# k2kobayashi/crank

Hardware: AMD Instinct MI355X
Metric: train frames/sec (higher is better)
Workload: dtype bf16; 1 GPU; vqvae trainer step (all sub-updates), VCC2020-shaped synthetic 80-dim mlfb, 64 utterances x 500 frames per GPU, 14 speakers; trainer=vqvae, global_batch=64, batch_len=500, parallelism=dp1

## Files before the change

### crank_amd/_lib.py

```python
import ctypes
import os
from .config import cfg
from ctypes import c_char_p, c_double, c_float, c_int, c_longlong, c_ulonglong, c_void_p

_HERE = os.path.dirname(os.path.abspath(__file__))
LIB_PATH = cfg.lib_path or os.path.join(_HERE, "libcrank_hip.so")
_lib = None

ERRORS = {1: "invalid argument", 2: "HIP runtime error", 3: "unsupported shape/configuration"}


class NetDesc(ctypes.Structure):
    _fields_ = [
        ("kind", c_int), ("in_ch", c_int), ("out_ch", c_int), ("kernel_size", c_int), ("layers", c_int),
        ("stacks", c_int), ("res_ch", c_int), ("gate_ch", c_int), ("skip_ch", c_int), ("aux_ch", c_int),
        ("conv_ch", c_int), ("causal", c_int), ("use_bias", c_int), ("slope", c_float), ("dropout", c_float),
    ]


COLLATE_MAX_STREAMS = 8


class CollateStream(ctypes.Structure):
    _fields_ = [("src", c_void_p), ("ld", c_int), ("col0", c_int), ("ncols", c_int), ("dst", c_void_p)]
# ... 35 lines not shown
    "crk_net_conv_info": (I, [P, I, ctypes.POINTER(c_longlong)]),
    "crk_net_saved_bytes": (LL, [P, I, I]),
    "crk_net_reserve": (I, [P, I, I]),
    "crk_net_scratch_bytes": (LL, [P, I, I]),
    "crk_debug_alloc_count": (LL, []),
    "crk_debug_net_paths": (I, [P, I, I]),
    "crk_debug_net_partials": (LL, [P, I, I, P, LL, P]),
    "crk_seed_next": (I, [P, P, P]),
    "crk_nets_wnorm_bwd": (I, [I, P, P]),
    "crk_nets_prepare": (I, [I, P, P, ULL, P, P]),
    "crk_nets_prepare_models": (I, [I, P, P, P, I, P, P]),
    "crk_net_forward": (I, [P, P, ULL, P, I, P, I, P, I, P, I, I, I, ULL, P]),
    "crk_net_backward": (I, [P, P, ULL, P, P, I, P, I, P, I, P, I, F, P, I, P, I, I, I, ULL, P]),
    "crk_net_backward_scaled": (I, [P, P, ULL, P, P, I, P, I, P, I, P, I, F, P, I, P, I, I, I, ULL, P, P, P]),
    "crk_net_embed_grad_supported": (I, [P, I, I, I]),
    "crk_net_backward_embed": (I, [P, P, ULL, P, P, I, P, I, P, I, P, I, F, P, I, I, I, ULL, P, LL, I, I, I, P, P]),
    "crk_vq_forward": (I, [P, I, P, I, I, I, P, P, I, P, I, P]),
    "crk_vq_forward_fused": (I, [P, I, P, I, P, I, P, I, I, I, P, P, I, P, I, P, P, P, P, P]),
    "crk_vq_image_bytes": (LL, [I, I]),
    "crk_vq_image_build_multi": (I, [I, P, P, I, P, P]),
    "crk_vq_ema_scratch_bytes": (LL, [I, I, I]),
    "crk_vq_ema_stats": (I, [P, I, P, I, I, I, P, P, P, P]),
    "crk_vq_ema_apply": (I, [P, P, P, P, P, I, I, D, D, P]),
    "crk_vq_ema_partial": (I, [P, I, P, I, I, I, P, P]),
    "crk_vq_ema_reduce_multi": (I, [I, P, P, P, P, P, P, P]),
    "crk_vq_ema_apply_multi": (I, [I, P, P, P, P, P, P, P, D, D, P]),
    "crk_vq_ema_partial_multi": (I, [I, P, P, P, P, P, P, P, P]),
    "crk_vq_ema_reduce_size_multi": (I, [I, P, P, P, P, P, P, P, D, D, P]),
    "crk_vq_ema_blend_multi": (I, [I, P, P, P, P, P, P, D, P]),
    "crk_vq_ema_blend_image_multi": (I, [I, P, P, P, P, P, P, D, P, P]),
# ... 152 lines not shown
```

### crank_amd/config.py

```python
import contextlib
import os
import types

_get = os.environ.get


def _flag(name, default):
    v = _get(name)
    return default if v is None else v not in ("0", "")


def _read():
    return types.SimpleNamespace(
        precision=_get("CRANK_AMD_PRECISION", "bf16"),
        lib_path=_get("CRANK_AMD_LIB") or None,
        default_yaml=_get("CRANK_DEFAULT_YAML") or None,
        overlap_c=int(_get("CRANK_AMD_OVERLAP_C", "3") or 0),
        separate_ce=_flag("CRANK_AMD_SEPARATE_CE", False),
        separate_commit=_flag("CRANK_AMD_SEPARATE_COMMIT", False),
        recon_dense=_flag("CRANK_AMD_RECON_DENSE", False),
        stft_two_pass=_flag("CRANK_AMD_STFT_TWO_PASS", False),
        cond_sums=_flag("CRANK_AMD_COND_SUMS", True),
        force_dist=_flag("CRANK_AMD_FORCE_DIST", False),
        dist_backend=_get("CRANK_AMD_DIST_BACKEND") or None,
        dp_graph_collectives=_flag("CRANK_AMD_DP_GRAPH_COLLECTIVES", True),
        capture_mode=_get("CRANK_AMD_CAPTURE_MODE", "thread_local"),
        test_refuse_capture_rank=_get("CRANK_AMD_TEST_REFUSE_CAPTURE_RANK"),
    )


cfg = _read()


def reload():
    cfg.__dict__.update(_read().__dict__)


# ... 17 lines not shown
```

### crank_amd/csrc/conv_kernels.h

```cpp
#pragma once
#include <vector>

#include "runtime.h"

#define CRK_TM 128

enum { MODE_PLAIN = 0, MODE_RESFWD = 1, MODE_BWDA = 2 };

struct ConvP {
  const float* xa; int lda; int cinA; float scaleA;
  const float* xb; int ldb; int cinB; float scaleB;
  int act_in; float slope;
  float drop_p; unsigned long long drop_seed;
  const unsigned long long* drop_seed_ptr;
  int cin, cin_pad;
  const float* xc; int ldc; int cinC; int cinC_pad;
  const uint16_t* w_hi; const uint16_t* w_lo;
  const uint16_t* wc_hi; const uint16_t* wc_lo;
  const uint16_t* w2_hi; const uint16_t* w2_lo;
  const float* bias; const float* bias2a; const float* bias2b;
  int cout, cout_pad, ktaps, dil, off0;
  int B, T, tiles_per_utt;
  float* y; int ldy; int accumulate; int act_out; float out_scale;
  const float* dmask; int ldm; int dmask_act;
// ... 61 lines not shown
  float drop_p; unsigned long long drop_seed; const unsigned long long* drop_seed_ptr;
  int o_xlo, o_zhi, o_zlo, o_chi, o_clo, o_whi, o_wlo, o_bias, o_tab, w_bytes, lds_bytes;
  int nw;
  int dbg;
  int ft, fh;
  int ft1;
  int o_zs, o_cs;
  int o_xf;
  const float* x_in; int ldx_in, in_ch, kp_first;
  long long f_first, b_first;
  long long f_h1, b_h1, f_h2, b_h2;
  float* y; int ldy, out_ch; float head_scale;
  uint16_t* fin_hi; uint16_t* head_hi;
  long long ts_stride;
  int cs_stride;
};
struct PsLayer {
  long long w_off;
  long long b_off;
  int rows, rows_pad;
  int kp;
  int k, dil, off0;
  int epi;
  int mask_w;
  long long mask_plane;
  long long save_plane;
  long long f_off;
};
struct PsP {
  const float* x; int ldx, cin; float in_scale; int in_act;
// ... 133 lines not shown
```

### crank_amd/csrc/net.hip

```cpp
#include <math.h>
#include <stdlib.h>
#include <string.h>

#include <deque>
#include <vector>

#include "conv_kernels.h"

#include "../../include/crank_hip.h"

enum { ROLE_FIRST = 0, ROLE_CONV = 1, ROLE_AUX = 2, ROLE_OUT = 3, ROLE_SKIP = 4, ROLE_LAST1 = 5, ROLE_LAST2 = 6, ROLE_PLAIN = 7 };

struct ConvMeta {
  int role, layer, dilation;
};

static bool g_may_alloc = false;
static long long g_net_allocs = 0;
static hipError_t net_malloc_(void** p, size_t bytes) {
  if (!g_may_alloc) return hipErrorInvalidValue;
  g_net_allocs++;
  return hipMalloc(p, bytes);
}
#define NET_MALLOC(pp, bytes) net_malloc_(reinterpret_cast<void**>(pp), (bytes))
// ... 632 lines not shown
    if (t.saved != saved) continue;
    if (t.B == B && t.T == T && t.mode == want && (want != 2 || t.x3f == expects_x3f)) {
      if (t.fused == fused) return CRK_OK;
      fprintf(stderr, "[crank_hip] crk_net_backward: the %s kernels would read a workspace the %s forward wrote (flags 0x%x, B %d, T %d)\n",
              fused ? "fused" : "per-layer", t.fused ? "fused" : "per-layer", flags, B, T);
      return CRK_ERR_ARG;
    }
    fprintf(stderr, "[crank_hip] crk_net_backward: flags 0x%x (plane layout %d%s, B %d, T %d) do not match the forward that wrote this "
                    "workspace (layout %d%s, B %d, T %d): CRK_FLAG_PRECISE pairs with CRK_FLAG_PRECISE, CRK_FLAG_PRECISE | CRK_FLAG_BWD_PLAIN "
                    "with CRK_FLAG_FWD_PRECISE, plain with plain\n", flags, want, expects_x3f ? " x3f" : "", B, T, t.mode, t.x3f ? " x3f" : "", t.B, t.T);
    return CRK_ERR_ARG;
  }
  return CRK_OK;
}

struct FwdIo {
  const float* params; const float* x; int ldx; const float* c; int ldc; float* y; int ldy; float* saved; int B, T; hipStream_t s;
};
enum { FWD_CHAIN, FWD_CHAIN_LAYERS, FWD_FOLDED, FWD_FUSED, FWD_LAYERS };
static int fwd_form(const Net* n, const Route& rt, const Call& k, bool x3f, int* form) {
  if (n->d.kind == 2) { *form = rt.fused ? FWD_CHAIN : FWD_CHAIN_LAYERS; return CRK_OK; }
  const bool io16 = k.in16 && k.out16;
  if ((x3f || rt.gen_split) && !io16) {
    fprintf(stderr, "[crank_hip] crk_net_forward: x / y must be 16-byte aligned with row strides that are multiples of 4 floats\n");
    return CRK_ERR_ARG;
  }
  if (x3f || (rt.fold_fwd && io16)) *form = FWD_FOLDED;
  else if (rt.gen_split) return CRK_ERR_UNSUPPORTED;
  else *form = rt.fused ? FWD_FUSED : FWD_LAYERS;
  return CRK_OK;
}

// ... 50 lines not shown
  sp.xb_lo = b16 + gf.xb_lo; sp.zb_lo = b16 + gf.zb_lo; sp.tb_lo = b16 + gf.tb_lo; sp.sg_lo = b16 + gf.sg_lo;
  if (n->d.aux_ch > 0) sp.cb_lo = b16 + gf.cb_lo;
  return sp;
}
static int fwd_folded(const Net* n, const Route& rt, const Call& k, const FwdIo& a, bool x3f) {
  const crk_net_desc& d = n->d;
  const ConvEntry& ef = n->ents[n->idx_first];
  const ConvEntry& e1 = n->ents[n->idx_last1];
  const ConvEntry& e2 = n->ents[n->idx_last2];
  StackP sp = stack_fwd_params(n, k, a, false);
  sp.x_in = a.x; sp.ldx_in = a.ldx; sp.in_ch = d.in_ch; sp.kp_first = ef.fw_kp;
  sp.f_first = ef.fr_off; sp.b_first = ef.off_b;
  sp.f_h1 = e1.fr_off; sp.b_h1 = e1.off_b; sp.f_h2 = e2.fr_off; sp.b_h2 = e2.off_b;
  sp.y = a.y; sp.ldy = a.ldy; sp.out_ch = d.out_ch; sp.head_scale = (float)sqrt(1.0 / n->L);
  if (x3f || rt.gen_split) sp.ts_stride = ts_plane_stride((long long)a.B * a.T);
  if (x3f) { RUN(stack2x_fwd_plan(sp)); return launch_stack2x_fwd(sp, a.s); }
  RUN(stack2_fwd_plan(sp));
  return launch_stack2_fwd(sp, a.s);
}
static int fwd_fused(const Net* n, const Shape* r, const Call& k, const FwdIo& a) {
  const crk_net_desc& d = n->d;
  const Route& rt = r->route[k.precise];
  const long long N = (long long)a.B * a.T;
  const GatedF32 lay = gated_f32(n, N);
  const GatedB16 gf = gated_b16(n, N);
  uint16_t* b16 = reinterpret_cast<uint16_t*>(a.saved + saved_f32_floats(n, N));
  PsP f = ps_base(n, a.B, a.T, a.params);
  f.x = a.x; f.ldx = a.ldx; f.cin = d.in_ch; f.y = a.saved + lay.x; f.ldy = 64; f.L = 1;
  if (k.keep) { f.save_hi = b16 + gf.f_hi; f.save_lo = b16 + gf.f_lo; }
  RUN(pstack_go(r, 0, f, k.precise, a.s));
// ... 37 lines not shown
    }
    p.w2_hi = n->whi + eo.fw_off; p.w2_lo = n->wlo + eo.fw_off;
    p.bias2a = eo.off_b >= 0 ? a.params + eo.off_b : nullptr;
    p.bias2b = es.off_b >= 0 ? a.params + es.off_b : nullptr;
    p.skip = SKIP; p.skip_init = (l == 0);
    p.sv_ta = a.saved + lay.ta + l * P; p.sv_sb = a.saved + lay.sb + l * P; p.sv_z = a.saved + lay.z + l * P;
    RUN(conv_go(p, MODE_RESFWD, k.precise, a.s));
  }
  ConvP h1 = conv_fw(n, a.B, a.T, n->ents[n->idx_last1], a.params, SKIP, 64, H1, 64);
  h1.scaleA = (float)sqrt(1.0 / L); h1.act_in = head_act;
  RUN(conv_go(h1, MODE_PLAIN, k.precise, a.s));
  ConvP h2 = conv_fw(n, a.B, a.T, n->ents[n->idx_last2], a.params, H1, 64, a.y, a.ldy);
  h2.act_in = head_act;
  return conv_go(h2, MODE_PLAIN, k.precise, a.s);
}
extern "C" int crk_net_forward(void* h, const float* params, unsigned long long version, const float* x, int ldx,
                               const float* c, int ldc, float* y, int ldy, float* saved, int B, int T, int flags,
                               unsigned long long seed, void* stream) {
  Net* n = (Net*)h;
  if (!n || !params || !x || !y || B <= 0 || T <= 0) return CRK_ERR_ARG;
  const FwdIo a = {.params = params, .x = x, .ldx = ldx, .c = c, .ldc = ldc, .y = y, .ldy = ldy, .saved = saved, .B = B, .T = T,
                   .s = (hipStream_t)stream};
  const Call k = call_facts(flags, seed, true, x, ldx, y, ldy, nullptr, nullptr);
  const Shape* r = find_shape(n, B, T);
  if (!r) return not_reserved("crk_net_forward");
  const Route rt = call_route(r, k);
  const bool x3f = k.mode == 2 && r->route[0].x3f;
  RUN(ensure_prepared(n, params, version, a.s));
  if (n->d.kind != 2 && (!saved || (n->d.aux_ch > 0 && !c))) return CRK_ERR_ARG;
  int form;
  RUN(fwd_form(n, rt, k, x3f, &form));
  tag_forward(n, saved, B, T, k, x3f, form != FWD_LAYERS && form != FWD_CHAIN_LAYERS);
  switch (form) {
    case FWD_CHAIN: return fwd_chain(n, r, k, a);
    case FWD_CHAIN_LAYERS: return fwd_chain_layers(n, k, a);
    case FWD_FOLDED: return fwd_folded(n, rt, k, a, x3f);
    case FWD_FUSED: return fwd_fused(n, r, k, a);
  }
  return fwd_layers(n, k, a);
}

static int stack_cpg(const Net* n, int B, int T) {
  const int ncpu = (T + 63) / 64;
  const int groups = crk_sw().wg_groups;
  const int gsz = (B + groups - 1) / groups;
  int cpg = gsz * ncpu;
  if (crk_sw().wg_fill && n->d.kind != 2 && n->L > 0 && 256 / n->L > groups) {
    const int fill = 256 / n->L;
    const int c = (B * ncpu + fill - 1) / fill;
    if (c >= 1 && c < cpg) cpg = c;
  }
  return cpg < 1 ? 1 : cpg;
}
static int stack_groups(const Net* n, int B, int T) {
// ... 597 lines not shown
```

### crank_amd/csrc/stack2_kernels.hip

```cpp
#include "conv_kernels.h"

#include "stack_common.h"

#define S2_NCU 256
#define S2_PAIR_FACTOR 1.0


template <int KT, int AKC, int FT, int R, int FH, bool DROP, bool FOLD>
__device__ __forceinline__ void s2_wave(const StackP& p, unsigned char* smem, const int rb) {
  constexpr int XS = SK_XS, NT = 256 * FH;
  const int tid = threadIdx.x, lane = tid & 63, l31 = lane & 31, half = lane >> 5;
  const int wave = __builtin_amdgcn_readfirstlane(tid >> 6);
  const int mt = wave & 3, fh = FH > 1 ? wave >> 2 : 0;
  const bool res_wave = mt < 2;
  const int b = blockIdx.x / p.tiles_per_utt, tile = blockIdx.x - b * p.tiles_per_utt;
  const int t0 = tile * p.tmo;
  const long nbase = (long)b * p.T;
  const long P = (long)p.B * p.T * 64;
  SK_PROF_BEGIN()

  unsigned char* xs = smem;
  unsigned char* zs = smem + p.o_zs;
  unsigned char* cs = smem + p.o_cs;
  StackLayer* lay_s = reinterpret_cast<StackLayer*>(smem + p.o_tab);
  float* bias_s = reinterpret_cast<float*>(smem + p.o_bias);

  int row[FT], voff_st[FT], voff_b[FT];
  unsigned rmask[FT];
  bool rin[FT];
  const bool save_b = p.xb_hi != nullptr;
  const int ch_st = 32 * (mt & 1) + 4 * half;
#pragma unroll
  for (int ft = 0; ft < FT; ft++) {
    row[ft] = rb + ft * 32 + l31;
// ... 28 lines not shown
      xq[u] = __builtin_amdgcn_raw_buffer_load_b128(rxi, on ? (int)(((nbase + t) * p.ldx_in + c4) * 4) : SK_OOB, 0, 0);
      xrow += xdr; xcol += xdc;
      if (xcol >= ppr) { xcol -= ppr; xrow++; }
    }
    if (res_wave) {
      const int KF = p.kp_first >> 4;
#pragma unroll
      for (int kc = 0; kc < 8; kc++) awf[kc] = S2_WLOAD(p.f_first + (mt * KF + (kc < KF ? kc : 0)) * 512);
    }
#pragma unroll
    for (int q = 0; q < 4; q++)
      bfq[q] = (res_wave && p.b_first >= 0) ? *reinterpret_cast<const sk_f32x4*>(p.params + p.b_first + 32 * mt + 8 * q + 4 * half) : sk_f32x4{0.f, 0.f, 0.f, 0.f};
  }
  constexpr int CNQ = R * 16, CPER = AKC > 0 ? (CNQ + NT - 1) / NT : 1;
  float av[CPER][4];
  if (AKC > 0) {
#pragma unroll
    for (int it = 0; it < CPER; it++) {
      const int idx = tid + it * NT, r = idx >> 4, c4 = (idx & 15) << 2;
      const int tt = t0 - p.hl + r;
      const bool on = idx < CNQ && tt >= 0 && tt < p.T;
      const long n = nbase + tt;
#pragma unroll
      for (int j = 0; j < 4; j++) av[it][j] = (on && c4 + j < p.aux_ch) ? p.c[n * p.ldc + c4 + j] : 0.f;
    }
  }
  SK_T(12)
  constexpr int NBI = 16 * 256 / NT;
  float bv[NBI];
#pragma unroll
  for (int k = 0; k < NBI; k++) {
// ... 427 lines not shown
  } else if (!res_wave) {
    const __amdgpu_buffer_rsrc_t r_sk = sk_rsrc(p.skip, P);
#pragma unroll
    for (int ft = 0; ft < FT; ft++)
#pragma unroll
      for (int q = 0; q < 4; q++) {
        sk_u32x4 v;
#pragma unroll
        for (int j = 0; j < 4; j++) v[j] = sk_f2u(st[ft][4 * q + j]);
        __builtin_amdgcn_raw_buffer_store_b128(v, r_sk, voff_st[ft] + q * 32, 0, 0);
      }
  }
  SK_PROF_END(7)
}

template <int KT, int AKC, int FT, int FH, bool DROP, bool FOLD, int FT1 = FT>
__global__ __launch_bounds__(256 * FH, 2) void stack2_fwd_kernel(const StackP p) {
  extern __shared__ __attribute__((aligned(16))) unsigned char smem[];
  constexpr int R = FH > 1 ? 32 * (FT + FT1) : 32 * FT;
  const int fh = FH > 1 ? __builtin_amdgcn_readfirstlane((int)threadIdx.x >> 8) : 0;
  if constexpr (FT1 == FT) {
    s2_wave<KT, AKC, FT, R, FH, DROP, FOLD>(p, smem, fh * 32 * FT);
  } else {
    if (fh == 0) s2_wave<KT, AKC, FT, R, FH, DROP, FOLD>(p, smem, 0);
    else s2_wave<KT, AKC, FT1, R, FH, DROP, FOLD>(p, smem, 32 * FT);
  }
}

int stack2_fwd_plan(StackP& p) {
  if ((p.ktaps != 3 && p.ktaps != 5) || p.max_off > SK_GUARD || p.aux_ch > 64 || p.L > 16) return CRK_ERR_UNSUPPORTED;
  if (p.ktaps == 3 && p.aux_ch > 0) return CRK_ERR_UNSUPPORTED;
  static int cfg_env = -1;
  if (cfg_env < 0) cfg_env = crk_sw().s2_cfg;
  static const int shapes[3][3] = {{2, 2, 2}, {3, 2, 2}, {3, 2, 3}};
  int best = -1; double best_cost = 0;
  for (int i = 0; i < 3; i++) {
    const int ft = shapes[i][0], fh = shapes[i][1], ft1 = shapes[i][2];
    const int code = ft1 == ft ? ft * 10 + fh : (ft * 10 + fh) * 10 + ft1;
    if (cfg_env && cfg_env != code) continue;
    if (ft1 != ft && (p.ktaps != 3 || p.drop_p > 0.f)) continue;
// ... 13 lines not shown
  p.tmo = ceil_div(p.T, p.tiles_per_utt);
  int off = (SK_GUARD * 2 + R) * SK_XS;
  p.o_zs = off; off += R * SK_XS;
  p.o_cs = off; if (p.aux_ch > 0) off += R * SK_XS;
  p.o_bias = off; off += p.L * 256 * 4;
  p.o_tab = off; off += p.L * (int)sizeof(StackLayer);
  off = (off + 15) & ~15;
  if (p.x_in) {
    if (p.kp_first < 16 || p.kp_first > 128 || (p.kp_first & 15)) return CRK_ERR_UNSUPPORTED;
    p.o_xf = off; off += R * (p.kp_first * 2 + 16);
  }
  p.lds_bytes = (off + 15) & ~15;
  return p.lds_bytes <= (p.fh == 1 ? 80 : 160) * 1024 ? CRK_OK : CRK_ERR_UNSUPPORTED;
}

template <int KT, int AKC, bool DROP, bool FOLD>
static int s2_launch_shape(const StackP& p, dim3 grid, hipStream_t s) {
#define S2_GO(FTV, FHV)                                                                                              \
  {                                                                                                                  \
    CRK_RAISE_LDS_ONCE(160 * 1024, stack2_fwd_kernel<KT, AKC, FTV, FHV, DROP, FOLD>)                                 \
    hipLaunchKernelGGL((stack2_fwd_kernel<KT, AKC, FTV, FHV, DROP, FOLD>), grid, dim3(256 * FHV), p.lds_bytes, s, p);       \
  }
  if (p.ft == 2) S2_GO(2, 2) else if (p.ft1 == 0) S2_GO(3, 2)
  else if constexpr (KT == 3 && !DROP) {
    CRK_RAISE_LDS_ONCE(160 * 1024, stack2_fwd_kernel<KT, AKC, 3, 2, DROP, FOLD, 2>)
    hipLaunchKernelGGL((stack2_fwd_kernel<KT, AKC, 3, 2, DROP, FOLD, 2>), grid, dim3(512), p.lds_bytes, s, p);
  } else return CRK_ERR_UNSUPPORTED;
#undef S2_GO
  return CRK_OK;
}

int launch_stack2_fwd(const StackP& p, hipStream_t s) {
  dim3 grid(p.B * p.tiles_per_utt);
  const double nfr = (double)p.B * p.T;
  conv_prof_bytes(1, nfr * (256.0 + 4.0 * p.aux_ch + 256.0 + (p.xb_hi ? 512.0 * p.L + 2.0 * (p.aux_ch > 0 ? p.aux_pad : 0) : 0.0)));
  conv_prof_begin(1, 2.0 * nfr * (p.L * (128.0 * (64.0 * p.ktaps + p.aux_ch) + 128.0 * 64.0) +
                                   (p.x_in ? 64.0 * p.in_ch + 64.0 * 64.0 + 64.0 * p.out_ch : 0.0)), s);
  const int akc = p.aux_ch > 0 ? (p.aux_ch + 15) / 16 : 0;
  int rc = CRK_OK;
  const bool fold = p.x_in != nullptr;
#define S2_DISPATCH(KTV, AKCV) (fold ? s2_launch_shape<KTV, AKCV, false, true>(p, grid, s) : s2_launch_shape<KTV, AKCV, false, false>(p, grid, s))
  if (p.ktaps == 3) rc = S2_DISPATCH(3, 0);
  else if (p.drop_p > 0.f) {
    if (akc || fold) return CRK_ERR_UNSUPPORTED;
    rc = s2_launch_shape<5, 0, true, false>(p, grid, s);
  } else if (akc == 0) rc = S2_DISPATCH(5, 0);
  else if (akc == 1) rc = S2_DISPATCH(5, 1);
  else if (akc <= 3) rc = S2_DISPATCH(5, 3);
  else rc = S2_DISPATCH(5, 4);
#undef S2_DISPATCH
  conv_prof_end(1, s);
  if (rc != CRK_OK) return rc;
  CRK_CHECK_LAUNCH();
  return CRK_OK;
}
```

### crank_amd/net/module/vqvae2.py

```python
import torch

from ... import ops, parallel
from .flat import FlatModel
from .mlfb import LogMelFilterBankLayer
from .pwg import KIND_GENERATOR, MAX_CHANNELS, HipStack


class Quantizer:

    def __init__(self, owner, prefix, emb_dim, emb_size, decay=0.99, eps=1e-5, ema_flag=False, bdt_flag=False):
        self.owner, self.prefix = owner, prefix
        self.emb_dim, self.emb_size = emb_dim, emb_size
        self.decay, self.eps, self.ema_flag, self.bdt_flag = decay, eps, ema_flag, bdt_flag
        self.cb_offset = None
        self.training = True
        self.bucket, self.slot = None, 0
        self._img, self._img_epoch = None, -1

    def entries(self, base):
        self.cb_offset = base
        return [(self.prefix + "embedding.weight", base, (self.emb_size, self.emb_dim))]

    @property
    def n_params(self):
# ... 275 lines not shown
            q.training = mode
        return self

    @property
    def spkr_table(self):
        o = self.emb_offset
        return self.flat.data[o: o + self.spkr_size * self.emb_size].view(self.spkr_size, self.emb_size)

    def spkr_embedding(self, h):
        return ops.concat_embed(None, None, self.spkr_table, h, self, self.emb_offset, self.flat)

    def _get_dec_h(self, dec_h, spkrvec):
        a, b = dec_h if isinstance(dec_h, (tuple, list)) else (dec_h, None)
        if spkrvec is not None:
            if torch.is_grad_enabled() and ops.embed_owned_ok(self.decoders[0].net, a, b, spkrvec):
                return ops.concat_embed_owned(a, b, self.spkr_table, spkrvec, self, self.emb_offset)
            return ops.concat_embed(a, b, self.spkr_table, spkrvec, self, self.emb_offset, self.flat)
        return dec_h if b is None else torch.cat([a, b], dim=-1)

    def _pre(self, x):
        return self.preprocess_layer(x) if self.conf["use_raw"] else x

    def encode(self, x, enc_h=None):
        out = []
        cur = x
        dims = self.conf["emb_dim"][: self.conf["n_vq_stacks"]]
        ebuf = torch.empty(x.shape[0], x.shape[1], sum(dims), device=x.device, dtype=torch.float32)
        col = 0
        for n in range(self.conf["n_vq_stacks"]):
            cur = self.encoders[n](cur, c=enc_h if n == 0 else None, out=(ebuf, col))
            col += dims[n]
# ... 103 lines not shown
```

### crank_amd/ops.py

```python
import ctypes

import torch

from . import _lib
from .config import cfg
from ._lib import check, ptr, stream_ptr

_PRECISION = cfg.precision


def set_precision(name):
    global _PRECISION
    if name not in ("bf16", "bf16x3", "bf16x3f"):
        raise ValueError(f"unknown precision {name!r} (bf16 | bf16x3 | bf16x3f)")
    _PRECISION = name


def get_precision():
    return _PRECISION


CRK_FLAG_PRECISE = 1
CRK_FLAG_NO_PARAM_GRAD = 2
CRK_FLAG_NO_SAVE = 4
# ... 95 lines not shown
        key = (B, T, _PRECISION)
        v = self._saved_bytes.get(key)
        if v is None:
            check(_lib.lib().crk_net_reserve(self.handle, B, T), "crk_net_reserve")
            v = self._saved_bytes[key] = _lib.lib().crk_net_saved_bytes(self.handle, B, T)
        return v

    def embed_grad_supported(self, B, T):
        key = ("embed", B, T, _PRECISION)
        v = self._saved_bytes.get(key)
        if v is None:
            self.saved_bytes(B, T)
            v = self._saved_bytes[key] = bool(_lib.lib().crk_net_embed_grad_supported(self.handle, B, T, _flags(backward=True)))
        return v

    def __del__(self):
        try:
            if getattr(self, "handle", None):
                _lib.lib().crk_net_destroy(self.handle)
                self.handle = None
        except Exception:
            pass


class _NetFn(torch.autograd.Function):

    @staticmethod
    def forward(ctx, x, c, flat, net, owner, offset, dx_scale, no_save=False, ybuf=None, ycol=0, emb=None):
        L = _lib.lib()
        B, T = x.shape[0], x.shape[1]
        if emb is not None and not (c is not None and emb.run == T and net.embed_grad_supported(B, T)):
            raise RuntimeError("conditioning built by concat_embed_owned fed to a net that cannot own its table gradient")
        xk, ldx = _rows(x)
        ck, ldc = (None, 0) if c is None else _rows(c)
        if ybuf is None:
            y = torch.empty(B, T, net.out_ch, device=x.device, dtype=torch.float32)
        else:
            y = ybuf[..., ycol: ycol + net.out_ch]
        ldy = y.stride(1)
        nbytes = net.saved_bytes(B, T)
        saved = torch.empty(max(nbytes // 4, 1), device=x.device, dtype=torch.float32)
        seed_t = net.next_seed() if net.dropout > 0 else None
        params = flat.data_ptr() + 4 * offset
        check(
            L.crk_net_forward(net.handle, params, owner.version, ptr(xk), ldx, ptr(ck), ldc, ptr(y), ldy,
                              ptr(saved), B, T, _flags(no_save=no_save) | (CRK_FLAG_SEED_ON_DEVICE if seed_t is not None else 0), ptr(seed_t),
                              stream_ptr()),
            "crk_net_forward",
        )
        ctx.net, ctx.owner, ctx.offset, ctx.dx_scale, ctx.seed = net, owner, offset, dx_scale, seed_t
        ctx.precision = _PRECISION
        ctx.ld = (ldx, ldc)
        ctx.version = owner.version
        ctx.save_for_backward(xk, ck if ck is not None else torch.empty(0, device=x.device), flat)
        ctx.saved_ws = saved
        ctx.has_c = c is not None
        ctx.emb = emb
        return y

    @staticmethod
    def backward(ctx, dy):
        L = _lib.lib()
        net, owner = ctx.net, ctx.owner
        xk, ck, flat = ctx.saved_tensors
# ... 751 lines not shown
                  "crk_weighted_sum_bwd")
        return (None, None) + tuple(grads[i] for i in range(len(ws)))


def weighted_sum(terms, weights, constant=0.0):
    return _WeightedSumFn.apply(tuple(weights), float(constant), *terms)


def _label_runs(idx):
    B, T = idx.shape
    if T > 1 and idx.stride(1) == 0 and (B == 1 or idx.stride(0) == T):
        return idx, T
    return idx.contiguous(), 1


def _concat_embed_fwd(a, b, table, idx):
    L = _lib.lib()
    B, T = idx.shape
    ak, lda = (None, 0) if a is None else _rows(a)
    bk, ldb = (None, 0) if b is None else _rows(b)
    ca = 0 if a is None else a.shape[-1]
    cb = 0 if b is None else b.shape[-1]
    E = table.shape[1]
    out = torch.empty(B, T, ca + cb + E, device=idx.device, dtype=torch.float32)
    ik, run = _label_runs(idx)
    check(L.crk_concat_embed_run(ptr(ak), lda, ca, ptr(bk), ldb, cb, ptr(table), E, ptr(ik), run, B * T, ptr(out),
                                 ca + cb + E, stream_ptr()), "crk_concat_embed_run")
    return out, ik, run, (ca, cb, E)


class _ConcatEmbedFn(torch.autograd.Function):

    @staticmethod
    def forward(ctx, a, b, table, idx, owner, tab_offset, flat):
        out, ik, run, (ca, cb, E) = _concat_embed_fwd(a, b, table, idx)
        B, T = idx.shape
        ctx.geom = (ca, cb, E, table.shape[0], run, B * T)
        ctx.owner, ctx.tab_offset = owner, tab_offset
        ctx.save_for_backward(ik)
        return out

    @staticmethod
    def backward(ctx, dout):
# ... 5 lines not shown
            ctx.owner.grads_clean = False
            g = ctx.owner.grad_flat[ctx.tab_offset: ctx.tab_offset + rows * E]
            scratch = torch.empty(L.crk_embed_bwd_scratch_floats(N, E, rows), device=dk.device, dtype=torch.float32)
            check(L.crk_embed_bwd_run(ptr(dk), ld, ca + cb, E, ptr(ik), run, N, rows, ptr(g), ptr(scratch), stream_ptr()),
                  "crk_embed_bwd_run")
        da = dk[..., :ca] if (ca and ctx.needs_input_grad[0]) else None
        db = dk[..., ca:ca + cb] if (cb and ctx.needs_input_grad[1]) else None
        return da, db, None, None, None, None, None


def concat_embed(a, b, table, idx, owner=None, tab_offset=0, flat=None):
    return _ConcatEmbedFn.apply(a, b, table, idx, owner, tab_offset, flat)


class EmbedCond:
    __slots__ = ("idx", "run", "c0", "E", "rows", "owner", "tab_offset")


def embed_owned_ok(net, a, b, idx):
    if not cfg.cond_sums or idx.dim() != 2:
        return False
    if (a is not None and a.requires_grad) or (b is not None and b.requires_grad):
        return False
    B, T = idx.shape
    return _label_runs(idx)[1] == T and net.embed_grad_supported(B, T)


def concat_embed_owned(a, b, table, idx, owner, tab_offset):
    with torch.no_grad():
        out, ik, run, (ca, cb, E) = _concat_embed_fwd(a, b, table, idx)
    e = EmbedCond()
    e.idx, e.run, e.c0, e.E, e.rows, e.owner, e.tab_offset = ik, run, ca + cb, E, table.shape[0], owner, tab_offset
    out._crk_embed = e
    return out


def adam_step(flat, grad, exp_avg, exp_avg_sq, lr_dev, step_dev, beta1=0.9, beta2=0.999, eps=1e-8, clear_grads=False,
              defer_bump=False):
    check(_lib.lib().crk_adam_step(ptr(flat), ptr(grad), ptr(exp_avg), ptr(exp_avg_sq), flat.numel(), ptr(lr_dev),
                                   ptr(step_dev), beta1, beta2, eps, (1 if clear_grads else 0) | (2 if defer_bump else 0),
                                   stream_ptr()), "crk_adam_step")


def adam_step_multi(blocks, beta1=0.9, beta2=0.999, eps=1e-8, clear_grads=False, defer_bump=False):
    rec = (_lib.AdamBlock * len(blocks))()
    for r, (flat, grad, m, v, lr_dev, step_dev) in zip(rec, blocks):
# ... 38 lines not shown
```

### include/crank_hip.h

```cpp
#ifndef CRANK_HIP_H
#define CRANK_HIP_H
#ifdef __cplusplus
extern "C" {
#endif

#define CRK_OK 0
#define CRK_ERR_ARG 1
#define CRK_ERR_HIP 2
#define CRK_ERR_UNSUPPORTED 3

#define CRK_FLAG_PRECISE 1
#define CRK_FLAG_NO_PARAM_GRAD 2
#define CRK_FLAG_NO_SAVE 4
#define CRK_FLAG_DEFER_WNORM 8

#define CRK_FLAG_SEED_ON_DEVICE 16
#define CRK_FLAG_FWD_PRECISE 32
#define CRK_FLAG_BWD_PLAIN 64

typedef struct crk_net_desc {
  int kind;
  int in_ch, out_ch, kernel_size, layers, stacks;
  int res_ch, gate_ch, skip_ch, aux_ch;
  int conv_ch;
// ... 2 lines not shown
  float slope;
  float dropout;
} crk_net_desc;

void* crk_net_create(const crk_net_desc* desc);
void crk_net_destroy(void* net);
long long crk_net_param_count(void* net);
int crk_net_conv_count(void* net);
int crk_net_conv_info(void* net, int i, long long* out9);
long long crk_net_saved_bytes(void* net, int B, int T);
int crk_net_reserve(void* net, int B, int T);
long long crk_net_scratch_bytes(void* net, int B, int T);
int crk_net_forward(void* net, const float* params, unsigned long long version, const float* x, int ldx,
                    const float* c, int ldc, float* y, int ldy, float* saved, int B, int T, int flags,
                    unsigned long long seed, void* stream);
int crk_net_backward(void* net, const float* params, unsigned long long version, float* grads, const float* x,
                     int ldx, const float* c, int ldc, const float* dy, int lddy, float* dx, int lddx, float dx_scale,
                     float* dc, int lddc, const float* saved, int B, int T, int flags, unsigned long long seed,
                     void* stream);
int crk_net_backward_scaled(void* net, const float* params, unsigned long long version, float* grads, const float* x,
                            int ldx, const float* c, int ldc, const float* dy, int lddy, float* dx, int lddx, float dx_scale,
                            float* dc, int lddc, const float* saved, int B, int T, int flags, unsigned long long seed,
                            const float* dy_num, const float* dy_den, void* stream);
int crk_net_embed_grad_supported(void* net, int B, int T, int flags);
int crk_net_backward_embed(void* net, const float* params, unsigned long long version, float* grads, const float* x, int ldx,
                           const float* c, int ldc, const float* dy, int lddy, float* dx, int lddx, float dx_scale,
                           const float* saved, int B, int T, int flags, unsigned long long seed, const long long* idx,
                           long long run, int c0, int E, int n_rows, float* dtable, void* stream);

int crk_seed_next(unsigned long long* state, unsigned long long* out, void* stream);
// ... 304 lines not shown
```

Before: 22.51 million frames/s.

## Fuse speaker-embedding concat gather into stacked decoder forward kernel

Instead of materializing the concatenated conditioning tensor (encoder outputs plus speaker embedding) with a separate concat kernel, the decoder's folded stack2 forward kernel now reads the two encoder parts and the embedding table row directly when it loads aux inputs. A placeholder NaN-expanded tensor stands in for the unbuilt conditioning, and the code falls back to the explicit concat when the gather path is unsupported. This removes one kernel launch and a B*T*aux_ch write/read, at the cost of a new template instantiation, extra per-element branching in the aux load, and risk if any consumer touches the placeholder tensor.

Result: no change. 22.48 million frames/s (median of 2 runs) (-0.1%).

```diff
diff --git a/crank_amd/_lib.py b/crank_amd/_lib.py
--- a/crank_amd/_lib.py
+++ b/crank_amd/_lib.py
@@ -73,6 +73,8 @@
     "crk_net_backward": (I, [P, P, ULL, P, P, I, P, I, P, I, P, I, F, P, I, P, I, I, I, ULL, P]),
     "crk_net_backward_scaled": (I, [P, P, ULL, P, P, I, P, I, P, I, P, I, F, P, I, P, I, I, I, ULL, P, P, P]),
     "crk_net_embed_grad_supported": (I, [P, I, I, I]),
+    "crk_net_forward_embed": (I, [P, P, ULL, P, I, P, I, I, P, I, I, P, I, P, LL, I, P, I, P, I, I, I, ULL, P]),
+    "crk_net_embed_gather_supported": (I, [P, I, I, I]),
     "crk_net_backward_embed": (I, [P, P, ULL, P, P, I, P, I, P, I, P, I, F, P, I, I, I, ULL, P, LL, I, I, I, P, P]),
     "crk_vq_forward": (I, [P, I, P, I, I, I, P, P, I, P, I, P]),
     "crk_vq_forward_fused": (I, [P, I, P, I, P, I, P, I, I, I, P, P, I, P, I, P, P, P, P, P]),
diff --git a/crank_amd/config.py b/crank_amd/config.py
--- a/crank_amd/config.py
+++ b/crank_amd/config.py
@@ -21,6 +21,7 @@
         recon_dense=_flag("CRANK_AMD_RECON_DENSE", False),
         stft_two_pass=_flag("CRANK_AMD_STFT_TWO_PASS", False),
         cond_sums=_flag("CRANK_AMD_COND_SUMS", True),
+        cond_gather=_flag("CRANK_AMD_COND_GATHER", True),
         force_dist=_flag("CRANK_AMD_FORCE_DIST", False),
         dist_backend=_get("CRANK_AMD_DIST_BACKEND") or None,
         dp_graph_collectives=_flag("CRANK_AMD_DP_GRAPH_COLLECTIVES", True),
diff --git a/crank_amd/csrc/conv_kernels.h b/crank_amd/csrc/conv_kernels.h
--- a/crank_amd/csrc/conv_kernels.h
+++ b/crank_amd/csrc/conv_kernels.h
@@ -99,6 +99,8 @@
   uint16_t* fin_hi; uint16_t* head_hi;
   long long ts_stride;
   int cs_stride;
+  const float* c2; int ldc2, ca, cb;
+  const float* emb_table; const long long* emb_idx; long long emb_run; int emb_c0, emb_E, emb_rows;
 };
 struct PsLayer {
   long long w_off;
diff --git a/crank_amd/csrc/net.hip b/crank_amd/csrc/net.hip
--- a/crank_amd/csrc/net.hip
+++ b/crank_amd/csrc/net.hip
@@ -670,8 +670,10 @@
   return CRK_OK;
 }
 
+struct CondGather { const float* c2; int ldc2, ca, cb; const float* table; const long long* idx; long long run; int E, n_rows; };
 struct FwdIo {
   const float* params; const float* x; int ldx; const float* c; int ldc; float* y; int ldy; float* saved; int B, T; hipStream_t s;
+  const CondGather* cg;
 };
 enum { FWD_CHAIN, FWD_CHAIN_LAYERS, FWD_FOLDED, FWD_FUSED, FWD_LAYERS };
 static int fwd_form(const Net* n, const Route& rt, const Call& k, bool x3f, int* form) {
@@ -752,6 +754,11 @@
   sp.f_h1 = e1.fr_off; sp.b_h1 = e1.off_b; sp.f_h2 = e2.fr_off; sp.b_h2 = e2.off_b;
   sp.y = a.y; sp.ldy = a.ldy; sp.out_ch = d.out_ch; sp.head_scale = (float)sqrt(1.0 / n->L);
   if (x3f || rt.gen_split) sp.ts_stride = ts_plane_stride((long long)a.B * a.T);
+  if (a.cg) {
+    const CondGather& g = *a.cg;
+    sp.c2 = g.c2; sp.ldc2 = g.ldc2; sp.ca = g.ca; sp.cb = g.cb;
+    sp.emb_table = g.table; sp.emb_idx = g.idx; sp.emb_run = g.run; sp.emb_c0 = g.ca + g.cb; sp.emb_E = g.E; sp.emb_rows = g.n_rows;
+  }
   if (x3f) { RUN(stack2x_fwd_plan(sp)); return launch_stack2x_fwd(sp, a.s); }
   RUN(stack2_fwd_plan(sp));
   return launch_stack2_fwd(sp, a.s);
@@ -819,23 +826,23 @@
   h2.act_in = head_act;
   return conv_go(h2, MODE_PLAIN, k.precise, a.s);
 }
-extern "C" int crk_net_forward(void* h, const float* params, unsigned long long version, const float* x, int ldx,
-                               const float* c, int ldc, float* y, int ldy, float* saved, int B, int T, int flags,
-                               unsigned long long seed, void* stream) {
+static int net_forward_impl(void* h, unsigned long long version, int flags, unsigned long long seed, const FwdIo& a) {
   Net* n = (Net*)h;
-  if (!n || !params || !x || !y || B <= 0 || T <= 0) return CRK_ERR_ARG;
-  const FwdIo a = {.params = params, .x = x, .ldx = ldx, .c = c, .ldc = ldc, .y = y, .ldy = ldy, .saved = saved, .B = B, .T = T,
-                   .s = (hipStream_t)stream};
-  const Call k = call_facts(flags, seed, true, x, ldx, y, ldy, nullptr, nullptr);
-  const Shape* r = find_shape(n, B, T);
+  if (!n || !a.params || !a.x || !a.y || a.B <= 0 || a.T <= 0) return CRK_ERR_ARG;
+  const Call k = call_facts(flags, seed, true, a.x, a.ldx, a.y, a.ldy, nullptr, nullptr);
+  const Shape* r = find_shape(n, a.B, a.T);
   if (!r) return not_reserved("crk_net_forward");
   const Route rt = call_route(r, k);
   const bool x3f = k.mode == 2 && r->route[0].x3f;
-  RUN(ensure_prepared(n, params, version, a.s));
-  if (n->d.kind != 2 && (!saved || (n->d.aux_ch > 0 && !c))) return CRK_ERR_ARG;
   int form;
+  if (a.cg) {
+    if (k.precise || x3f || !rt.usums || n->d.kind == 2 || fwd_form(n, rt, k, x3f, &form) != CRK_OK || form != FWD_FOLDED)
+      return CRK_ERR_UNSUPPORTED;
+  }
+  RUN(ensure_prepared(n, a.params, version, a.s));
+  if (n->d.kind != 2 && (!a.saved || (n->d.aux_ch > 0 && !a.c && !a.cg))) return CRK_ERR_ARG;
   RUN(fwd_form(n, rt, k, x3f, &form));
-  tag_forward(n, saved, B, T, k, x3f, form != FWD_LAYERS && form != FWD_CHAIN_LAYERS);
+  tag_forward(n, a.saved, a.B, a.T, k, x3f, form != FWD_LAYERS && form != FWD_CHAIN_LAYERS);
   switch (form) {
     case FWD_CHAIN: return fwd_chain(n, r, k, a);
     case FWD_CHAIN_LAYERS: return fwd_chain_layers(n, k, a);
@@ -843,6 +850,32 @@
     case FWD_FUSED: return fwd_fused(n, r, k, a);
   }
   return fwd_layers(n, k, a);
+}
+extern "C" int crk_net_forward(void* h, const float* params, unsigned long long version, const float* x, int ldx,
+                               const float* c, int ldc, float* y, int ldy, float* saved, int B, int T, int flags,
+                               unsigned long long seed, void* stream) {
+  const FwdIo a = {.params = params, .x = x, .ldx = ldx, .c = c, .ldc = ldc, .y = y, .ldy = ldy, .saved = saved, .B = B, .T = T,
+                   .s = (hipStream_t)stream, .cg = nullptr};
+  return net_forward_impl(h, version, flags, seed, a);
+}
+extern "C" int crk_net_embed_gather_supported(void* h, int B, int T, int flags) {
+  Net* n = (Net*)h;
+  if (!n || B <= 0 || T <= 0 || (flags & CRK_FLAG_PRECISE) || n->d.kind == 2) return 0;
+  const Route rt = route_at(n, B, T, false);
+  return rt.usums && rt.fold_fwd ? 1 : 0;
+}
+extern "C" int crk_net_forward_embed(void* h, const float* params, unsigned long long version, const float* x, int ldx,
+                                     const float* a, int lda, int ca, const float* b, int ldb, int cb, const float* table, int E,
+                                     const long long* idx, long long run, int n_rows, float* y, int ldy, float* saved, int B, int T,
+                                     int flags, unsigned long long seed, void* stream) {
+  Net* n = (Net*)h;
+  if (!n || !table || !idx || run != T || ca < 0 || cb < 0 || E < 1 || n_rows < 1 || (ca > 0 && (!a || lda < ca)) ||
+      (cb > 0 && (!b || ldb < cb)) || ca + cb + E != n->d.aux_ch)
+    return CRK_ERR_ARG;
+  const CondGather cg = {b, ldb, ca, cb, table, idx, run, E, n_rows};
+  const FwdIo io = {.params = params, .x = x, .ldx = ldx, .c = a, .ldc = lda, .y = y, .ldy = ldy, .saved = saved, .B = B, .T = T,
+                    .s = (hipStream_t)stream, .cg = &cg};
+  return net_forward_impl(h, version, flags, seed, io);
 }
 
 static int stack_cpg(const Net* n, int B, int T) {
diff --git a/crank_amd/csrc/stack2_kernels.hip b/crank_amd/csrc/stack2_kernels.hip
--- a/crank_amd/csrc/stack2_kernels.hip
+++ b/crank_amd/csrc/stack2_kernels.hip
@@ -6,7 +6,7 @@
 #define S2_PAIR_FACTOR 1.0
 
 
-template <int KT, int AKC, int FT, int R, int FH, bool DROP, bool FOLD>
+template <int KT, int AKC, int FT, int R, int FH, bool DROP, bool FOLD, bool GATHER>
 __device__ __forceinline__ void s2_wave(const StackP& p, unsigned char* smem, const int rb) {
   constexpr int XS = SK_XS, NT = 256 * FH;
   const int tid = threadIdx.x, lane = tid & 63, l31 = lane & 31, half = lane >> 5;
@@ -18,6 +18,7 @@
   const long nbase = (long)b * p.T;
   const long P = (long)p.B * p.T * 64;
   SK_PROF_BEGIN()
+  const long long label = (AKC > 0 && GATHER) ? p.emb_idx[(long long)b * p.emb_run] : 0;
 
   unsigned char* xs = smem;
   unsigned char* zs = smem + p.o_zs;
@@ -76,7 +77,29 @@
   }
   constexpr int CNQ = R * 16, CPER = AKC > 0 ? (CNQ + NT - 1) / NT : 1;
   float av[CPER][4];
-  if (AKC > 0) {
+  if constexpr (AKC > 0 && GATHER) {
+    const int c4 = (tid & 15) << 2;
+    float tv[4];
+#pragma unroll
+    for (int j = 0; j < 4; j++) {
+      const int e = c4 + j - p.emb_c0;
+      tv[j] = (e >= 0 && e < p.emb_E && label >= 0 && label < p.emb_rows) ? p.emb_table[label * p.emb_E + e] : 0.f;
+    }
+#pragma unroll
+    for (int it = 0; it < CPER; it++) {
+      const int idx = tid + it * NT, r = idx >> 4;
+      const int tt = t0 - p.hl + r;
+      const bool on = idx < CNQ && tt >= 0 && tt < p.T;
+      const long n = nbase + tt;
+#pragma unroll
+      for (int j = 0; j < 4; j++) {
+        const int col = c4 + j;
+        float v = tv[j];
+        if (col < p.emb_c0) v = !on ? 0.f : (col < p.ca ? p.c[n * p.ldc + col] : p.c2[n * p.ldc2 + col - p.ca]);
+        av[it][j] = on ? v : 0.f;
+      }
+    }
+  } else if constexpr (AKC > 0) {
 #pragma unroll
     for (int it = 0; it < CPER; it++) {
       const int idx = tid + it * NT, r = idx >> 4, c4 = (idx & 15) << 2;
@@ -534,16 +557,16 @@
   SK_PROF_END(7)
 }
 
-template <int KT, int AKC, int FT, int FH, bool DROP, bool FOLD, int FT1 = FT>
+template <int KT, int AKC, int FT, int FH, bool DROP, bool FOLD, int FT1 = FT, bool GATHER = false>
 __global__ __launch_bounds__(256 * FH, 2) void stack2_fwd_kernel(const StackP p) {
   extern __shared__ __attribute__((aligned(16))) unsigned char smem[];
   constexpr int R = FH > 1 ? 32 * (FT + FT1) : 32 * FT;
   const int fh = FH > 1 ? __builtin_amdgcn_readfirstlane((int)threadIdx.x >> 8) : 0;
   if constexpr (FT1 == FT) {
-    s2_wave<KT, AKC, FT, R, FH, DROP, FOLD>(p, smem, fh * 32 * FT);
+    s2_wave<KT, AKC, FT, R, FH, DROP, FOLD, GATHER>(p, smem, fh * 32 * FT);
   } else {
-    if (fh == 0) s2_wave<KT, AKC, FT, R, FH, DROP, FOLD>(p, smem, 0);
-    else s2_wave<KT, AKC, FT1, R, FH, DROP, FOLD>(p, smem, 32 * FT);
+    if (fh == 0) s2_wave<KT, AKC, FT, R, FH, DROP, FOLD, GATHER>(p, smem, 0);
+    else s2_wave<KT, AKC, FT1, R, FH, DROP, FOLD, GATHER>(p, smem, 32 * FT);
   }
 }
 
@@ -587,15 +610,15 @@
   return p.lds_bytes <= (p.fh == 1 ? 80 : 160) * 1024 ? CRK_OK : CRK_ERR_UNSUPPORTED;
 }
 
-template <int KT, int AKC, bool DROP, bool FOLD>
+template <int KT, int AKC, bool DROP, bool FOLD, bool GATHER = false>
 static int s2_launch_shape(const StackP& p, dim3 grid, hipStream_t s) {
 #define S2_GO(FTV, FHV)                                                                                              \
   {                                                                                                                  \
-    CRK_RAISE_LDS_ONCE(160 * 1024, stack2_fwd_kernel<KT, AKC, FTV, FHV, DROP, FOLD>)                                 \
-    hipLaunchKernelGGL((stack2_fwd_kernel<KT, AKC, FTV, FHV, DROP, FOLD>), grid, dim3(256 * FHV), p.lds_bytes, s, p);       \
+    CRK_RAISE_LDS_ONCE(160 * 1024, stack2_fwd_kernel<KT, AKC, FTV, FHV, DROP, FOLD, FTV, GATHER>)                    \
+    hipLaunchKernelGGL((stack2_fwd_kernel<KT, AKC, FTV, FHV, DROP, FOLD, FTV, GATHER>), grid, dim3(256 * FHV), p.lds_bytes, s, p); \
   }
   if (p.ft == 2) S2_GO(2, 2) else if (p.ft1 == 0) S2_GO(3, 2)
-  else if constexpr (KT == 3 && !DROP) {
+  else if constexpr (KT == 3 && !DROP && !GATHER) {
     CRK_RAISE_LDS_ONCE(160 * 1024, stack2_fwd_kernel<KT, AKC, 3, 2, DROP, FOLD, 2>)
     hipLaunchKernelGGL((stack2_fwd_kernel<KT, AKC, 3, 2, DROP, FOLD, 2>), grid, dim3(512), p.lds_bytes, s, p);
   } else return CRK_ERR_UNSUPPORTED;
@@ -612,7 +635,12 @@
   const int akc = p.aux_ch > 0 ? (p.aux_ch + 15) / 16 : 0;
   int rc = CRK_OK;
   const bool fold = p.x_in != nullptr;
-#define S2_DISPATCH(KTV, AKCV) (fold ? s2_launch_shape<KTV, AKCV, false, true>(p, grid, s) : s2_launch_shape<KTV, AKCV, false, false>(p, grid, s))
+  const bool gather = p.emb_table != nullptr;
+  if (gather && !(fold && akc > 0 && p.ktaps == 5 && p.drop_p == 0.f)) return CRK_ERR_UNSUPPORTED;
+#define S2_DISPATCH(KTV, AKCV)                                                                                        \
+  (fold ? ((AKCV) > 0 && gather ? s2_launch_shape<KTV, AKCV, false, true, ((AKCV) > 0)>(p, grid, s)                   \
+                                : s2_launch_shape<KTV, AKCV, false, true>(p, grid, s))                                \
+        : s2_launch_shape<KTV, AKCV, false, false>(p, grid, s))
   if (p.ktaps == 3) rc = S2_DISPATCH(3, 0);
   else if (p.drop_p > 0.f) {
     if (akc || fold) return CRK_ERR_UNSUPPORTED;
diff --git a/crank_amd/net/module/vqvae2.py b/crank_amd/net/module/vqvae2.py
--- a/crank_amd/net/module/vqvae2.py
+++ b/crank_amd/net/module/vqvae2.py
@@ -313,7 +313,7 @@
         a, b = dec_h if isinstance(dec_h, (tuple, list)) else (dec_h, None)
         if spkrvec is not None:
             if torch.is_grad_enabled() and ops.embed_owned_ok(self.decoders[0].net, a, b, spkrvec):
-                return ops.concat_embed_owned(a, b, self.spkr_table, spkrvec, self, self.emb_offset)
+                return ops.concat_embed_owned(a, b, self.spkr_table, spkrvec, self, self.emb_offset, net=self.decoders[0].net)
             return ops.concat_embed(a, b, self.spkr_table, spkrvec, self, self.emb_offset, self.flat)
         return dec_h if b is None else torch.cat([a, b], dim=-1)
 
diff --git a/crank_amd/ops.py b/crank_amd/ops.py
--- a/crank_amd/ops.py
+++ b/crank_amd/ops.py
@@ -133,6 +133,14 @@
             v = self._saved_bytes[key] = bool(_lib.lib().crk_net_embed_grad_supported(self.handle, B, T, _flags(backward=True)))
         return v
 
+    def embed_gather_supported(self, B, T):
+        key = ("gather", B, T, _PRECISION)
+        v = self._saved_bytes.get(key)
+        if v is None:
+            self.saved_bytes(B, T)
+            v = self._saved_bytes[key] = bool(_lib.lib().crk_net_embed_gather_supported(self.handle, B, T, _flags()))
+        return v
+
     def __del__(self):
         try:
             if getattr(self, "handle", None):
@@ -151,7 +159,6 @@
         if emb is not None and not (c is not None and emb.run == T and net.embed_grad_supported(B, T)):
             raise RuntimeError("conditioning built by concat_embed_owned fed to a net that cannot own its table gradient")
         xk, ldx = _rows(x)
-        ck, ldc = (None, 0) if c is None else _rows(c)
         if ybuf is None:
             y = torch.empty(B, T, net.out_ch, device=x.device, dtype=torch.float32)
         else:
@@ -161,12 +168,25 @@
         saved = torch.empty(max(nbytes // 4, 1), device=x.device, dtype=torch.float32)
         seed_t = net.next_seed() if net.dropout > 0 else None
         params = flat.data_ptr() + 4 * offset
-        check(
-            L.crk_net_forward(net.handle, params, owner.version, ptr(xk), ldx, ptr(ck), ldc, ptr(y), ldy,
-                              ptr(saved), B, T, _flags(no_save=no_save) | (CRK_FLAG_SEED_ON_DEVICE if seed_t is not None else 0), ptr(seed_t),
-                              stream_ptr()),
-            "crk_net_forward",
-        )
+        flags = _flags(no_save=no_save) | (CRK_FLAG_SEED_ON_DEVICE if seed_t is not None else 0)
+        gathered = False
+        if emb is not None and emb.parts is not None:
+            (ak, lda, ca), (bk, ldb, cb), table = emb.parts
+            rc = L.crk_net_forward_embed(net.handle, params, owner.version, ptr(xk), ldx, ptr(ak), lda, ca, ptr(bk), ldb, cb,
+                                         ptr(table), emb.E, ptr(emb.idx), emb.run, emb.rows, ptr(y), ldy, ptr(saved), B, T, flags,
+                                         ptr(seed_t), stream_ptr())
+            if rc == 3:
+                c = _concat_embed_launch(ak, lda, ca, bk, ldb, cb, table, emb.idx, emb.run, B, T)
+            else:
+                check(rc, "crk_net_forward_embed")
+                gathered = True
+        ck, ldc = (None, 0) if (c is None or gathered) else _rows(c)
+        if not gathered:
+            check(
+                L.crk_net_forward(net.handle, params, owner.version, ptr(xk), ldx, ptr(ck), ldc, ptr(y), ldy,
+                                  ptr(saved), B, T, flags, ptr(seed_t), stream_ptr()),
+                "crk_net_forward",
+            )
         ctx.net, ctx.owner, ctx.offset, ctx.dx_scale, ctx.seed = net, owner, offset, dx_scale, seed_t
         ctx.precision = _PRECISION
         ctx.ld = (ldx, ldc)
@@ -948,19 +968,28 @@
     return idx.contiguous(), 1
 
 
-def _concat_embed_fwd(a, b, table, idx):
-    L = _lib.lib()
-    B, T = idx.shape
+def _concat_embed_launch(ak, lda, ca, bk, ldb, cb, table, ik, run, B, T):
+    E = table.shape[1]
+    out = torch.empty(B, T, ca + cb + E, device=ik.device, dtype=torch.float32)
+    check(_lib.lib().crk_concat_embed_run(ptr(ak), lda, ca, ptr(bk), ldb, cb, ptr(table), E, ptr(ik), run, B * T, ptr(out),
+                                          ca + cb + E, stream_ptr()), "crk_concat_embed_run")
+    return out
+
+
+def _concat_embed_parts(a, b, idx):
     ak, lda = (None, 0) if a is None else _rows(a)
     bk, ldb = (None, 0) if b is None else _rows(b)
     ca = 0 if a is None else a.shape[-1]
     cb = 0 if b is None else b.shape[-1]
-    E = table.shape[1]
-    out = torch.empty(B, T, ca + cb + E, device=idx.device, dtype=torch.float32)
     ik, run = _label_runs(idx)
-    check(L.crk_concat_embed_run(ptr(ak), lda, ca, ptr(bk), ldb, cb, ptr(table), E, ptr(ik), run, B * T, ptr(out),
-                                 ca + cb + E, stream_ptr()), "crk_concat_embed_run")
-    return out, ik, run, (ca, cb, E)
+    return (ak, lda, ca), (bk, ldb, cb), ik, run
+
+
+def _concat_embed_fwd(a, b, table, idx):
+    B, T = idx.shape
+    (ak, lda, ca), (bk, ldb, cb), ik, run = _concat_embed_parts(a, b, idx)
+    out = _concat_embed_launch(ak, lda, ca, bk, ldb, cb, table, ik, run, B, T)
+    return out, ik, run, (ca, cb, table.shape[1])
 
 
 class _ConcatEmbedFn(torch.autograd.Function):
@@ -996,7 +1025,7 @@
 
 
 class EmbedCond:
-    __slots__ = ("idx", "run", "c0", "E", "rows", "owner", "tab_offset")
+    __slots__ = ("idx", "run", "c0", "E", "rows", "owner", "tab_offset", "parts")
 
 
 def embed_owned_ok(net, a, b, idx):
@@ -1008,10 +1037,27 @@
     return _label_runs(idx)[1] == T and net.embed_grad_supported(B, T)
 
 
-def concat_embed_owned(a, b, table, idx, owner, tab_offset):
-    with torch.no_grad():
-        out, ik, run, (ca, cb, E) = _concat_embed_fwd(a, b, table, idx)
+_NAN = {}
+
+
+def _unbuilt(device, shape):
+    if device not in _NAN:
+        _NAN[device] = torch.full((1,), float("nan"), device=device, dtype=torch.float32)
+    return _NAN[device].expand(shape)
+
+
+def concat_embed_owned(a, b, table, idx, owner, tab_offset, net=None):
+    B, T = idx.shape
     e = EmbedCond()
+    if net is not None and cfg.cond_gather and net.embed_gather_supported(B, T):
+        pa, pb, ik, run = _concat_embed_parts(a, b, idx)
+        ca, cb, E = pa[2], pb[2], table.shape[1]
+        e.parts = (pa, pb, table)
+        out = _unbuilt(idx.device, (B, T, ca + cb + E))
+    else:
+        with torch.no_grad():
+            out, ik, run, (ca, cb, E) = _concat_embed_fwd(a, b, table, idx)
+        e.parts = None
     e.idx, e.run, e.c0, e.E, e.rows, e.owner, e.tab_offset = ik, run, ca + cb, E, table.shape[0], owner, tab_offset
     out._crk_embed = e
     return out
diff --git a/include/crank_hip.h b/include/crank_hip.h
--- a/include/crank_hip.h
+++ b/include/crank_hip.h
@@ -40,6 +40,11 @@
 int crk_net_forward(void* net, const float* params, unsigned long long version, const float* x, int ldx,
                     const float* c, int ldc, float* y, int ldy, float* saved, int B, int T, int flags,
                     unsigned long long seed, void* stream);
+int crk_net_forward_embed(void* net, const float* params, unsigned long long version, const float* x, int ldx,
+                          const float* a, int lda, int ca, const float* b, int ldb, int cb, const float* table, int E,
+                          const long long* idx, long long run, int n_rows, float* y, int ldy, float* saved, int B, int T,
+                          int flags, unsigned long long seed, void* stream);
+int crk_net_embed_gather_supported(void* net, int B, int T, int flags);
 int crk_net_backward(void* net, const float* params, unsigned long long version, float* grads, const float* x,
                      int ldx, const float* c, int ldc, const float* dy, int lddy, float* dx, int lddx, float dx_scale,
                      float* dc, int lddc, const float* saved, int B, int T, int flags, unsigned long long seed,
```
